# TimoLassmann/tagdust

Hardware: AMD Instinct MI355X
Metric: reads/s (150 bp, 8-barcode arch) (higher is better)
Workload: dtype f32

## Files before the change

### tagdust_amd/csrc/td_api.hip

```cpp
#include <math.h>
#include <stdarg.h>
#include <stdlib.h>
#include <string.h>
#include <time.h>
#include <unistd.h>

#include <mutex>
#include <thread>

#include "../../include/tagdust_model.h"
#include "td_ctx.h"
#include "td_rnadust.h"
#include "td_stats.h"

static float g_logsum[TD_LOGSUM_SIZE];
static bool g_logsum_ready = false;
static std::string g_create_error;

static void init_logsum_host()
{
	if (g_logsum_ready) return;
	for (int i = 0; i < TD_LOGSUM_SIZE; i++) g_logsum[i] = (float)log(1.0 + exp((double)-i / (double)1000.0f));
	g_logsum_ready = true;
}
// ... 405 lines not shown
static int slot_events(td_ctx* c, TdSlot& s)
{
	if (s.ev_k0) return TD_OK;
	HIPCHK(c, hipEventCreate(&s.ev_k0));
	HIPCHK(c, hipEventCreate(&s.ev_k1));
	HIPCHK(c, hipEventCreateWithFlags(&s.ev_up, hipEventDisableTiming));
	HIPCHK(c, hipEventCreateWithFlags(&s.ev_done, hipEventDisableTiming));
	HIPCHK(c, hipEventCreateWithFlags(&s.ev_down, hipEventDisableTiming));
	HIPCHK(c, hipEventCreateWithFlags(&s.ev_pack, hipEventDisableTiming));
	HIPCHK(c, hipEventCreateWithFlags(&s.ev_hits, hipEventDisableTiming));
	return TD_OK;
}

static void slot_release(TdSlot& s)
{
	void* dev[] = { s.d_raw, s.d_offs, s.d_read_at, s.d_keys, s.d_vals, s.d_sort_tmp, s.d_packed, s.d_lens, s.d_art_left,
	                s.d_out, s.d_res, s.d_seq, s.d_lab, s.d_keepo, s.d_rle, s.d_runs, s.d_judged };
	for (void* p : dev) if (p) (void)hipFree(p);
	void* pinned[] = { s.h_raw, s.h_offs, s.h_res, s.h_seq, s.h_lab, s.h_keepo, s.h_rle };
	for (void* p : pinned) if (p) (void)hipHostFree(p);
	hipEvent_t ev[] = { s.ev_up, s.ev_k0, s.ev_k1, s.ev_done, s.ev_down, s.ev_pack, s.ev_hits };
	for (hipEvent_t e : ev) if (e) (void)hipEventDestroy(e);
	s = TdSlot();
}

static int hbm_free(td_ctx* c, size_t& free_b)
{
	size_t total_b = 0;
	HIPCHK(c, hipMemGetInfo(&free_b, &total_b));
	return TD_OK;
}
// ... 73 lines not shown
		if (l < 0 || l > 100000) { bad = i; break; }
		if (l > lmax) lmax = (int)l;
		if (l < lmin) lmin = (int)l;
	}
	if (bad >= 0) return fail(c, "td_batch_upload: read %lld has length %lld", (long long)bad, (long long)(offs[bad + 1] - offs[bad]));
	const int64_t n_bases = n > 0 ? offs[n] - base : 0;
	const int64_t n_tiles = (n + TD_WAVE - 1) / TD_WAVE;
	const TdLengthClasses lc = plan_length_classes(offs, n, lmin, lmax, n_tiles, c->spec.ready && with_workspace && c->length_classes);
	s.n_long = lc.n_long; s.lmax_small = lc.lmax_small;
	const int nw2 = (lmax + 15) / 16, nw1 = (lmax + 31) / 32;
	const bool sorted = n > 0 && lmin != lmax;

	const size_t n_packed = (size_t)(n_tiles * (int64_t)(nw2 + nw1) * TD_WAVE), n_lanes = (size_t)(n_tiles * TD_WAVE);
	const OutLayout ol = out_layout(n_tiles, lmax, nw1);
	if (ensure(c, &s.d_raw, &s.cap_raw, (size_t)n_bases) != TD_OK || ensure(c, &s.d_offs, &s.cap_offs, (size_t)(n + 1) * 8) != TD_OK ||
	    ensure(c, &s.d_packed, &s.cap_packed, n_packed * 4) != TD_OK || ensure(c, &s.d_lens, &s.cap_lens, n_lanes * 4) != TD_OK ||
	    ensure(c, &s.d_art_left, &s.cap_art_left, n_lanes) != TD_OK || ensure(c, &s.d_out, &s.cap_out, (size_t)ol.total) != TD_OK)
		return TD_FAIL;
	size_t sort_tmp = 0;
	if (sorted) {
		sort_tmp = td_stage_sort_temp_bytes(n, lmax);
		if (ensure(c, &s.d_read_at, &s.cap_read_at, (size_t)n * 4) != TD_OK || ensure(c, &s.d_keys, &s.cap_keys, (size_t)n * 8) != TD_OK ||
		    ensure(c, &s.d_vals, &s.cap_vals, (size_t)n * 4) != TD_OK || ensure(c, &s.d_sort_tmp, &s.cap_sort_tmp, sort_tmp) != TD_OK)
			return TD_FAIL;
	}
	s.lmax = lmax; s.nw2 = nw2; s.nw1 = nw1; s.n_tiles = (int32_t)n_tiles;
	if (with_workspace && ensure_workspace(c, s) != TD_OK) { s.n_tiles = 0; return TD_FAIL; }
	s.for_spec = with_workspace && c->spec.ready;
	s.n_tiles = 0;

	const void* src = (const uint8_t*)bases + base;
	s.raw_direct = n_bases > 0 && is_pinned(src);
	if (n_bases > 0 && !s.raw_direct) {
		if (ensure_pinned(c, &s.h_raw, &s.cap_h_raw, (size_t)n_bases) != TD_OK) return TD_FAIL;
		parallel_copy(c, s.h_raw, src, (size_t)n_bases);
		src = s.h_raw;
		s.raw_host = s.h_raw;
	} else if (n_bases > 0 && c->stable_input && s.pipelined) {
		s.raw_host = (const uint8_t*)src;
	}
	HIPCHK(c, hipMemcpyAsync(s.d_offs, s.h_offs, (size_t)(n + 1) * 8, hipMemcpyHostToDevice, up));
	if (n_bases > 0) HIPCHK(c, hipMemcpyAsync(s.d_raw, src, (size_t)n_bases, hipMemcpyHostToDevice, up));
	if (up != s.aux) {
		HIPCHK(c, hipEventRecord(s.ev_up, up));
		HIPCHK(c, hipStreamWaitEvent(s.aux, s.ev_up, 0));
	}
	if (sorted)
		HIPCHK(c, td_stage_sort(s.d_offs, n, lmax, s.d_read_at, s.d_keys, s.d_keys + n, s.d_vals, s.d_sort_tmp, sort_tmp, s.aux));
	TdStageBatch& b = s.sb;
	b = TdStageBatch{};
	b.raw = s.d_raw; b.offs = s.d_offs; b.n_reads = n; b.is_ascii = is_ascii;
	b.n_tiles = (int32_t)n_tiles; b.lmax = lmax; b.nw2 = nw2; b.nw1 = nw1;
	b.read_at = sorted ? s.d_read_at : nullptr;
	b.packed = s.d_packed; b.lens = s.d_lens; b.art_left = s.d_art_left;
	b.out_soa = s.d_out; b.soa_stride = ol.soa_stride;
	b.keep = (const uint32_t*)(s.d_out + ol.keep); b.labels = (const int8_t*)(s.d_out + ol.labels);
	HIPCHK(c, td_stage_pack(b, s.aux));
	if (s.aux != s.cs) {
		HIPCHK(c, hipEventRecord(s.ev_pack, s.aux));
		HIPCHK(c, hipStreamWaitEvent(s.cs, s.ev_pack, 0));
	}

	s.n_reads = n; s.n_bases = n_bases; s.n_tiles = (int32_t)n_tiles; s.is_ascii = is_ascii; s.sorted = sorted;
	s.staged = true;
	return TD_OK;
}

static int rle_capacity(const td_ctx* c)
{
	int cap = c->dev.h.S + 2 < c->dev.h.H ? c->dev.h.S + 2 : c->dev.h.H;
	if (c->rle_cap_forced > 0) cap = c->rle_cap_forced;
	return cap;
}

static int slot_rna_dust(td_ctx* c, TdSlot& s);

static int slot_count_hits(td_ctx* c, TdSlot& s, const int32_t* out_type)
{
	HIPCHK(c, td_stage_art_hits(out_type, s.n_reads, c->art_n, c->d_art_hits, s.cs));
// ... 12 lines not shown
	HIPCHK(c, hipSetDevice(c->device));
	s.reset_decoded();
	s.mode = mode;
	if (s.n_tiles == 0) { s.ran = true; s.last_ms = 0.0f; return TD_OK; }
	if (c->spec.ready && s.for_spec && c->match_len > 0 && !c->spec.window) {
		HIPCHK(c, sync_compute(c));
		if (spec_load_window_variant(c) != TD_OK) return TD_FAIL;
		if (!c->spec.ready) {
			s.n_long = 0; s.lmax_small = s.lmax;
			if (ensure_workspace(c, s) != TD_OK) return TD_FAIL;
			s.for_spec = false;
		}
	}
	const bool use_spec = c->spec.ready && s.for_spec;
	if (s.for_spec && !c->spec.ready) return fail(c, "td_run: the resident batch was staged for a specialised kernel that is no longer loaded (upload it again)");
	const OutLayout ol = out_layout(s.n_tiles, s.lmax, s.nw1);
	TdKernelArgs ka{};
	ka.hdr = c->dev.d_hdr; ka.cols = c->dev.d_cols; ka.hinfo = c->dev.d_hinfo;
	ka.pred_off = c->dev.d_pred_off; ka.pred_idx = c->dev.d_pred_idx; ka.logsum = c->d_logsum;
	ka.packed = s.d_packed; ka.lens = s.d_lens;
	ka.n_tiles = s.n_tiles; ka.n_slots = s.n_wave_slots; ka.lmax = s.lmax; ka.nw2 = s.nw2; ka.nw1 = s.nw1;
	ka.mode = mode; ka.threshold = c->threshold; ka.minlen = c->minlen; ka.dust = c->dust; ka.want_labels = 1;
	ka.win_start = c->match_start; ka.win_len = c->match_len;
	point_outputs(ka, s.d_out, ol);
	ka.counters = c->d_counters;
	ka.ws = s.wsi ? c->d_ws2 : c->d_ws; ka.lay = s.lay;
	if (c->art_n > 0 && mode == TD_MODE_GET_LABEL) {
		s.sb.art_threads = c->art_threads;
		s.sb.art_first = c->win_first; s.sb.art_total = c->win_total;
		HIPCHK(c, td_stage_art_left(s.sb, s.cs));
		ka.art_text = c->d_art_text; ka.art_index = c->d_art_index; ka.art_left = s.d_art_left;
		ka.art_n = c->art_n; ka.art_fe = c->art_fe;
	}
	if (c->poison) HIPCHK(c, hipMemsetAsync(ka.ws, 0xFF, (size_t)s.ws_bytes, s.cs));
	if (use_spec) {
		int32_t*& tn = s.wsi ? c->d_tile_next2 : c->d_tile_next;
		if (!tn) HIPCHK(c, hipMalloc((void**)&tn, 256));
		HIPCHK(c, hipMemsetAsync(tn, 0, sizeof(int32_t), s.cs));
	}
	HIPCHK(c, hipEventRecord(s.ev_k0, s.cs));
	if (use_spec) {
		TdSpecArgs sa = spec_args_from(ka);
		sa.lay = s.slay;
		sa.lmax = s.n_big > 0 ? s.lmax_small : s.lmax;
		sa.n_big = s.n_big; sa.lmax_big = s.lmax; sa.lay_big = s.slay_big; sa.out_lmax = s.lmax;
		if (mode == TD_MODE_GET_LABEL && want_labels && c->compact_egress) {
			const int cap = rle_capacity(c);
			const size_t words = (size_t)s.n_tiles * (size_t)cap * TD_WAVE + 1;
			if (ensure(c, &s.d_runs, &s.cap_runs, words * 4) != TD_OK) return TD_FAIL;
			if (c->poison) HIPCHK(c, hipMemsetAsync(s.d_runs, 0xFF, (words - 1) * 4, s.cs));
			HIPCHK(c, hipMemsetAsync(s.d_runs + words - 1, 0, 4, s.cs));
			sa.out_runs = s.d_runs; sa.rle_overflow = (int32_t*)(s.d_runs + words - 1); sa.rle_cap = cap;
			s.runs_cap = cap;
		}
		sa.prune = c->spec.d_prune; sa.prune_stride = c->spec.prune_stride;
		sa.tile_next = s.wsi ? c->d_tile_next2 : c->d_tile_next;
		HIPCHK(c, spec_launch(c, sa, s.cs));
// ... 6 lines not shown
	if (c->census.on && mode == TD_MODE_GET_LABEL && census_count_slot(c, s, ka.out_type, ka.out_labels) != TD_OK) return TD_FAIL;
	if (c->molecules.on && mode == TD_MODE_GET_LABEL && mol_slot_decoded(c, s, ka.out_type, ka.out_barcode, ka.out_finger, ka.out_labels) != TD_OK) return TD_FAIL;
	s.ran = true;
	s.last_ms = -1.0f;
	c->last_slot = (int)(&s - c->slots);
	return TD_OK;
}

static int slot_rna_dust(td_ctx* c, TdSlot& s)
{
	if (!s.staged) return fail(c, "td_run: no batch resident (td_batch_upload failed or was not called)");
	HIPCHK(c, hipSetDevice(c->device));
	s.reset_decoded();
	s.mode = TD_MODE_RNA_DUST;
	if (s.n_tiles == 0) { s.ran = true; s.last_ms = 0.0f; return TD_OK; }
	const OutLayout ol = out_layout(s.n_tiles, s.lmax, s.nw1);
	TdRnaDustArgs ra{};
	ra.packed = s.d_packed; ra.lens = s.d_lens; ra.n_tiles = s.n_tiles; ra.nw2 = s.nw2; ra.nw1 = s.nw1;
	ra.raw = s.d_raw; ra.offs = s.d_offs; ra.read_at = s.sorted ? s.d_read_at : nullptr; ra.n_reads = s.n_reads; ra.is_ascii = s.is_ascii;
	ra.dust = c->dust;
	if (c->art_n > 0) {
		s.sb.art_threads = c->art_threads;
		s.sb.art_first = c->win_first; s.sb.art_total = c->win_total;
		HIPCHK(c, td_stage_art_left(s.sb, s.cs));
		ra.art_pk = c->d_art_pk; ra.art_seq = c->d_art_seq; ra.art_left = s.d_art_left;
		ra.art_n = c->art_n; ra.art_fe = c->art_fe;
	}
	point_outputs(ra, s.d_out, ol);
	ra.counters = c->d_counters;
	HIPCHK(c, hipEventRecord(s.ev_k0, s.cs));
// ... 452 lines not shown
```

### tagdust_amd/csrc/td_batch_plan.cpp

```cpp
#include "td_batch_plan.h"

#include <vector>

int64_t align256(int64_t v) { return (v + 255) & ~(int64_t)255; }

void make_layout(TdWsLayout& L, int S, int H, int C, int lmax, int max_ncol)
{
	int64_t o = 0;
	L.codes = o; o = align256(o + (int64_t)(lmax + 2) * TD_WAVE);
	L.sb = o;    o = align256(o + (int64_t)(S + 1) * (lmax + 2) * TD_WAVE * 4);
	L.sf = o;    o = align256(o + (int64_t)(S + 1) * (lmax + 2) * TD_WAVE * 4);
	L.bw = o;    o = align256(o + (int64_t)C * lmax * TD_WAVE * 8);
	L.fwrow = o; o = align256(o + (int64_t)max_ncol * TD_WAVE * 8);
	L.dp = o;    o = align256(o + (int64_t)lmax * H * TD_WAVE * 4);
	L.path = o;  o = align256(o + (int64_t)lmax * H * TD_WAVE);
	L.acc = o;   o = align256(o + (int64_t)H * TD_WAVE * 4);
	L.total = o; o = align256(o + (int64_t)H * TD_WAVE * 4);
	L.dust = o;  o = align256(o + (int64_t)64 * TD_WAVE);
	L.slot_bytes = o;
}

OutLayout out_layout(int64_t n_tiles, int lmax, int nw1)
{
	OutLayout o;
// ... 13 lines not shown
	for (int64_t i = 0; i < n; i++) hist[(size_t)(offs[i + 1] - offs[i])]++;
	const int64_t t99 = n_tiles - 1 - (n_tiles + 99) / 100;
	const int64_t rank = t99 * TD_WAVE + TD_WAVE - 1;
	int64_t acc = 0;
	int l99 = lmax;
	for (int l = 0; l <= lmax; l++) { acc += hist[(size_t)l]; if (acc > rank) { l99 = l; break; } }
	if (l99 < 1) l99 = 1;
	if ((int64_t)lmax * 2 >= (int64_t)l99 * 3) {
		int64_t upto = 0;
		for (int l = 0; l <= l99; l++) upto += hist[(size_t)l];
		const int64_t first_long_tile = upto / TD_WAVE;
		lc.n_long = (int32_t)(n_tiles - first_long_tile);
		lc.lmax_small = l99;
	}
	return lc;
}

TdWsPlan plan_workspace(const TdWsRequest& rq, TdFreeMemFn free_mem, void* arg)
{
	TdWsPlan p;
	p.half_slots = rq.half_slots;
	int overlap = rq.overlap, wsi = rq.wsi;
	for (;;) {
		p.n_long = rq.n_long; p.lmax_small = rq.lmax_small;
		p.one_geometry = false;
		int64_t slot_bytes = rq.small_slot_bytes;
		const int wpb = rq.wpb;
		int64_t slots = rq.want_slots;
		if (slots > rq.n_tiles) slots = rq.n_tiles;
		if (slots < 1) slots = 1;
// ... 58 lines not shown
```

### tagdust_amd/csrc/td_batch_plan.h

```cpp
#pragma once
#include <stddef.h>
#include <stdint.h>

#include "td_device.h"

#ifndef TD_HIDDEN
#define TD_HIDDEN __attribute__((visibility("hidden")))
#endif

TD_HIDDEN int64_t align256(int64_t v);
TD_HIDDEN void make_layout(TdWsLayout& L, int S, int H, int C, int lmax, int max_ncol);
struct OutLayout { int64_t soa_stride, keep, labels, total; };
TD_HIDDEN OutLayout out_layout(int64_t n_tiles, int lmax, int nw1);

struct TdLengthClasses { int32_t n_long, lmax_small; };
TD_HIDDEN TdLengthClasses plan_length_classes(const int64_t* offs, int64_t n, int lmin, int lmax, int64_t n_tiles, bool wanted);

struct TdWsRequest {
	int64_t n_tiles = 0;
	int32_t n_long = 0, lmax_small = 0, lmax = 0;
	int64_t small_slot_bytes = 0, big_slot_bytes = 0;
	int wpb = 1;
	int64_t want_slots = 0;
	bool spec_ready = false, pipelined = false;
	int overlap = 0, pipeline_depth = 1;
	bool half_slots = false;
	int wsi = 0;
	size_t cap_ws = 0, cap_ws2 = 0;
	int ws_candidates = 1;
};
struct TdWsPlan {
// ... 13 lines not shown
```

### tagdust_amd/csrc/td_ctx.h

```cpp
#pragma once
#include <hip/hip_runtime.h>
#include <stdio.h>
#include <memory>
#include <string>
#include <vector>
#include "../../include/tagdust_hip.h"
#include "td_device.h"
#include "td_batch_plan.h"
#include "td_jit.h"
#include "td_stage.h"
#include "td_host_inner.h"
#include "td_census.h"
#include "td_molecules.h"

#define TD_HIDDEN __attribute__((visibility("hidden")))
#define TD_MAX_PIPELINE 4
#define TD_COUNTER_WORDS (TD_NUM_COUNTERS + TD_NUM_DIAG_COUNTERS)

struct TdRoute {
	hipStream_t cs = nullptr;
	hipStream_t aux = nullptr;
	hipStream_t fin = nullptr;
	int wsi = 0;
	bool pipelined = false;
};
struct TdStaged : TdRoute {
	int64_t n_reads = 0, n_bases = 0;
	int32_t n_tiles = 0, lmax = 0, nw2 = 0, nw1 = 0;
	int is_ascii = 0;
	bool sorted = false;
	bool staged = false;
	bool for_spec = false;
	bool raw_direct = false;
	const uint8_t* raw_host = nullptr;
	TdStageBatch sb{};
	TdWsLayout lay{};
	TdSpecLayout slay{};
	int32_t n_wave_slots = 0;
	int64_t ws_slot_bytes = 0;
	int32_t n_long = 0, lmax_small = 0, n_big = 0;
	TdSpecLayout slay_big{};
	int64_t ws_bytes = 0;
};
struct TdDecoded {
	int mode = 0;
	bool ran = false;
	float last_ms = -1.0f;
// ... 8 lines not shown
	int32_t rle_cap = 0;
	bool finished = false;
};
struct TdSlot : TdStaged, TdDecoded, TdFetch {
	int64_t ticket = 0;
	void reset_staged(const TdRoute& r) { static_cast<TdStaged&>(*this) = TdStaged(); static_cast<TdRoute&>(*this) = r; reset_decoded(); }
	void reset_decoded() { static_cast<TdDecoded&>(*this) = TdDecoded(); reset_fetch(); }
	void reset_fetch() { static_cast<TdFetch&>(*this) = TdFetch(); }
	uint8_t* d_raw = nullptr;      size_t cap_raw = 0;
	int64_t* d_offs = nullptr;     size_t cap_offs = 0;
	int32_t* d_read_at = nullptr;  size_t cap_read_at = 0;
	uint32_t* d_keys = nullptr;    size_t cap_keys = 0;
	int32_t* d_vals = nullptr;     size_t cap_vals = 0;
	uint8_t* d_sort_tmp = nullptr; size_t cap_sort_tmp = 0;
	uint32_t* d_packed = nullptr;  size_t cap_packed = 0;
	int32_t* d_lens = nullptr;     size_t cap_lens = 0;
	uint8_t* d_art_left = nullptr; size_t cap_art_left = 0;
	uint8_t* d_out = nullptr;      size_t cap_out = 0;
	uint8_t* d_res = nullptr;      size_t cap_res = 0;
	uint8_t* d_seq = nullptr;      size_t cap_seq = 0;
	int8_t*  d_lab = nullptr;      size_t cap_lab = 0;
	uint32_t* d_keepo = nullptr;   size_t cap_keepo = 0;
	uint32_t* d_rle = nullptr;     size_t cap_rle = 0;
	uint32_t* d_runs = nullptr;    size_t cap_runs = 0;
	int32_t* d_judged = nullptr;   size_t cap_judged = 0;
	uint32_t* h_keepo = nullptr;   size_t cap_h_keepo = 0;
	uint32_t* h_rle = nullptr;     size_t cap_h_rle = 0;
	uint8_t* h_raw = nullptr;      size_t cap_h_raw = 0;
	int64_t* h_offs = nullptr;     size_t cap_h_offs = 0;
	uint8_t* h_res = nullptr;      size_t cap_h_res = 0;
// ... 163 lines not shown
template <typename Args> static void point_labels(Args&, int8_t*, long) {}
template <typename Args>
static void point_outputs(Args& a, uint8_t* out, const OutLayout& ol)
{
	float* soa = (float*)out;
	const int64_t st = ol.soa_stride / 4;
	a.out_f = soa; a.out_b = soa + st; a.out_r = soa + 2 * st; a.out_bar = soa + 3 * st; a.out_q = soa + 4 * st;
	a.out_type = (int32_t*)(soa + 5 * st); a.out_barcode = (int32_t*)(soa + 6 * st); a.out_finger = (int32_t*)(soa + 7 * st);
	a.out_keep = (uint32_t*)(out + ol.keep);
	point_labels(a, (int8_t*)(out + ol.labels), 0);
}

static TdSpecArgs spec_args_from(const TdKernelArgs& ka)
{
	TdSpecArgs sa{};
	sa.logsum = ka.logsum; sa.packed = ka.packed; sa.lens = ka.lens;
	sa.n_tiles = ka.n_tiles; sa.n_slots = ka.n_slots; sa.lmax = ka.lmax; sa.nw2 = ka.nw2; sa.nw1 = ka.nw1;
	sa.mode = ka.mode; sa.threshold = ka.threshold; sa.minlen = ka.minlen; sa.dust = ka.dust;
	sa.win_start = ka.win_start; sa.win_len = ka.win_len;
	sa.out_f = ka.out_f; sa.out_b = ka.out_b; sa.out_r = ka.out_r; sa.out_bar = ka.out_bar; sa.out_q = ka.out_q;
	sa.out_type = ka.out_type; sa.out_barcode = ka.out_barcode; sa.out_finger = ka.out_finger;
	sa.out_keep = ka.out_keep; sa.out_labels = ka.out_labels; sa.counters = ka.counters;
	sa.art_text = ka.art_text; sa.art_index = ka.art_index; sa.art_left = ka.art_left; sa.art_n = ka.art_n; sa.art_fe = ka.art_fe;
	sa.ws = ka.ws;
	return sa;
}

TD_HIDDEN int spec_model_uploaded(td_ctx* c);
TD_HIDDEN int spec_handover(td_ctx* c, bool block);
TD_HIDDEN int spec_before_batch(td_ctx* c, int lmax);
TD_HIDDEN int spec_load_window_variant(td_ctx* c);
// ... 5 lines not shown
```

### tagdust_amd/csrc/td_device.h

```cpp
#pragma once
#include <stdint.h>

#define TD_WAVE 64
#define TD_LOGSUM_LIVE 15700

enum : uint32_t {
	TDF_MM = 1u << 0, TDF_MI = 1u << 1, TDF_MD = 1u << 2, TDF_II = 1u << 3, TDF_IM = 1u << 4,
	TDF_DD = 1u << 5, TDF_DM = 1u << 6, TDF_MSKIP = 1u << 7, TDF_ISKIP = 1u << 8,
	TDF_SM = 1u << 9, TDF_SI = 1u << 10,
};

struct TdCol {
	float    t[9];
	float    sM, sI;
	float    eM[5];
	float    eI[5];
	uint32_t flags;
	uint32_t pad[2];
};
static_assert(sizeof(TdCol) == 96, "TdCol layout");

struct TdSeg {
	int32_t n_hmm, n_col, col_off, hmm_off;
	float   skip;
// ... 49 lines not shown
	float*   __restrict__ out_q;
	int32_t* __restrict__ out_type;
	int32_t* __restrict__ out_barcode;
	int32_t* __restrict__ out_finger;
	uint32_t* __restrict__ out_keep;
	int8_t*  __restrict__ out_labels;
	unsigned long long* __restrict__ counters;
	const uint8_t*  __restrict__ art_text;
	const int32_t*  __restrict__ art_index;
	const uint8_t*  __restrict__ art_left;
	int32_t art_n, art_fe;
	uint8_t* __restrict__ ws;
	TdWsLayout lay;
};

struct TdSpecLayout {
	int64_t slot_bytes;
	int64_t codes;
	int64_t sb;
	int64_t sf;
	int64_t bw;
	int64_t dp;
	int64_t path;
	int64_t total;
	int64_t rs;
	int64_t bm;
	int64_t ba;
	int64_t acc;
	int64_t pmask;
};

struct TdSpecArgs {
	const float*  __restrict__ logsum;
	const uint32_t* __restrict__ packed;
	const int32_t*  __restrict__ lens;
	int32_t n_tiles, n_slots, lmax, nw2, nw1;
	int32_t mode;
	float   threshold;
	int32_t minlen, dust;
	int32_t win_start, win_len;
	int32_t prune_stride;
	float*   __restrict__ out_f;
	float*   __restrict__ out_b;
	float*   __restrict__ out_r;
	float*   __restrict__ out_bar;
	float*   __restrict__ out_q;
	int32_t* __restrict__ out_type;
	int32_t* __restrict__ out_barcode;
	int32_t* __restrict__ out_finger;
	uint32_t* __restrict__ out_keep;
// ... 18 lines not shown
```

### tagdust_amd/csrc/td_jit.hip

```cpp
#include <hip/hip_runtime.h>
#include <hip/hiprtc.h>
#include <math.h>
#include <stdio.h>
#include <string.h>
#include <stdlib.h>

#include <atomic>
#include <map>
#include <mutex>
#include <string>
#include <vector>

#include "../../include/tagdust_hip.h"
#include "td_device.h"
#include <unistd.h>
#include <sys/stat.h>
#include <sys/types.h>
#include "td_embedded_src.h"
#include "td_jit.h"

static std::string flit(float v)
{
	if (isinf(v)) return v < 0 ? "(-__builtin_inff())" : "__builtin_inff()";
	if (v != v) return "__builtin_nanf(\"\")";
// ... 285 lines not shown
{
	std::string src = "#ifndef __HIPCC_RTC__\n#include <hip/hip_runtime.h>\n#endif\n#include <stdint.h>\n";
	src += kSrcDeviceH;
	src += "\n";
	src += kSrcArtifact;
	src += "\n";
	src += td_spec_model_section(m, p, lsum_oob, window);
	src += kSrcSpecKernel;
	return src;
}

void td_spec_layout(TdSpecLayout& L, const TdSpecPlan& p, int lmax)
{
	auto al = [](int64_t v) { return (v + 255) & ~(int64_t)255; };
	int64_t o = 0;
	L.codes = o; o = al(o + (int64_t)(lmax + 2) * TD_WAVE);
	L.sb = o;    o = al(o + (int64_t)(p.S + 1) * (lmax + 2) * TD_WAVE * 4);
	L.sf = o;    o = al(o + (int64_t)(p.S + 1) * (lmax + 2) * TD_WAVE * 4);
	L.bw = o;    o = al(o + p.halves * lmax * TD_WAVE * 4 + 1024);
	L.dp = o;    o = al(o + (int64_t)lmax * p.H * TD_WAVE * 4);
	L.path = o;  o = al(o + (int64_t)lmax * ((p.H + 3) / 4) * TD_WAVE * 4);
	L.total = o; o = al(o + (int64_t)p.H * TD_WAVE * 4);
	L.rs = o;    o = al(o + (int64_t)2 * p.C * TD_WAVE * 4);
	L.bm = o;    o = al(o + (int64_t)(lmax + 2) * TD_WAVE * 4);
	L.ba = o;    o = al(o + (int64_t)(lmax + 2) * TD_WAVE);
	L.acc = o;   o = al(o + (int64_t)2 * p.H * TD_WAVE * 4);
	L.pmask = o; o = al(o + (int64_t)p.H * ((lmax + 31) / 32) * 4);
	L.slot_bytes = o;
}

static uint64_t fnv1a(const std::string& t)
// ... 171 lines not shown
```

### tagdust_amd/csrc/td_spec_host.hip

```cpp
#include <stdlib.h>
#include <algorithm>
#include <cmath>
#include <condition_variable>
#include <map>
#include <mutex>
#include <thread>

#include "td_ctx.h"

struct SpecJob {
	uint64_t key = 0;
	ModelCopy model;
	TdSpecPlan plan;
	int lsum_oob = 0, window = 0;
	std::mutex mu;
	std::condition_variable cv;
	bool done = false;
	int rc = TD_FAIL;
	std::vector<char> code;
	std::string log;
	std::thread th;
	void run()
	{
		std::vector<char> out;
// ... 70 lines not shown
	std::vector<uint8_t> codes((size_t)n_bases);
	(void)td_spec_probe(&c->model.d, codes.data(), n_bases, nullptr);
	const int n = TD_PROBE_READS, n_tiles = TD_PROBE_READS / TD_WAVE;
	int lmax = 1;
	for (int i = 0; i < n; i++) if (offs[(size_t)i + 1] - offs[(size_t)i] > lmax) lmax = (int)(offs[(size_t)i + 1] - offs[(size_t)i]);
	const int nw2 = (lmax + 15) / 16, nw1 = (lmax + 31) / 32;
	if (ensure_prune_tables(c, lmax) != TD_OK) return TD_FAIL;
	const TdModelHeader& h = c->dev.h;
	TdWsLayout glay{};
	make_layout(glay, h.S, h.H, h.C, lmax, h.max_ncol);
	TdSpecLayout slay{};
	td_spec_layout(slay, c->spec.plan, lmax);
	const int gwpb = td_kernel_block_threads() / TD_WAVE, swpb = c->spec.block / TD_WAVE;
	const int gslots = (n_tiles + gwpb - 1) / gwpb * gwpb, sslots = (n_tiles + swpb - 1) / swpb * swpb;
	const OutLayout ol = out_layout(n_tiles, lmax, nw1);
	int64_t o = 0;
	auto carve = [&](int64_t bytes) { const int64_t at = o; o = align256(o + bytes); return at; };
	const int64_t o_raw = carve(n_bases), o_offs = carve((int64_t)(n + 1) * 8), o_packed = carve((int64_t)n_tiles * (nw2 + nw1) * TD_WAVE * 4),
	              o_lens = carve((int64_t)n * 4), o_outa = carve(ol.total), o_outb = carve(ol.total),
	              o_cnt = carve((int64_t)2 * TD_COUNTER_WORDS * 8), o_cmp = carve(256), o_tile = carve(256);
	const int64_t small_bytes = o;
	const int64_t o_wsa = carve((int64_t)gslots * glay.slot_bytes), o_wsb = carve((int64_t)sslots * slay.slot_bytes);
	uint8_t* d = nullptr;
	HIPCHK(c, hipMalloc((void**)&d, (size_t)o));
	struct Free { uint8_t* p; ~Free() { (void)hipFree(p); } } free_{ d };
	hipStream_t st = c->stream;
	HIPCHK(c, hipMemsetAsync(d, 0, (size_t)small_bytes, st));
	HIPCHK(c, hipMemsetAsync(d + o_cmp, 0xFF, 256, st));
	HIPCHK(c, hipMemsetAsync(d + o_cmp, 0, 4, st));
	HIPCHK(c, hipMemsetAsync(d + o_wsa, 0xFF, (size_t)(o - o_wsa), st));
	HIPCHK(c, hipMemcpyAsync(d + o_raw, codes.data(), (size_t)n_bases, hipMemcpyHostToDevice, st));
	HIPCHK(c, hipMemcpyAsync(d + o_offs, offs.data(), (size_t)(n + 1) * 8, hipMemcpyHostToDevice, st));
	TdStageBatch sb{};
	sb.raw = d + o_raw; sb.offs = (const int64_t*)(d + o_offs); sb.n_reads = n; sb.is_ascii = 0;
	sb.n_tiles = n_tiles; sb.lmax = lmax; sb.nw2 = nw2; sb.nw1 = nw1;
	sb.read_at = nullptr;
	sb.packed = (uint32_t*)(d + o_packed); sb.lens = (int32_t*)(d + o_lens);
	HIPCHK(c, td_stage_pack(sb, st));
	unsigned long long* cnt_a = (unsigned long long*)(d + o_cnt);
	unsigned long long* cnt_b = cnt_a + TD_COUNTER_WORDS;
	TdKernelArgs ka{};
	ka.hdr = c->dev.d_hdr; ka.cols = c->dev.d_cols; ka.hinfo = c->dev.d_hinfo; ka.pred_off = c->dev.d_pred_off; ka.pred_idx = c->dev.d_pred_idx; ka.logsum = c->d_logsum;
	ka.packed = sb.packed; ka.lens = sb.lens;
	ka.n_tiles = n_tiles; ka.n_slots = gslots; ka.lmax = lmax; ka.nw2 = nw2; ka.nw1 = nw1;
	ka.mode = TD_MODE_GET_LABEL; ka.threshold = TD_PROBE_THRESHOLD; ka.minlen = TD_PROBE_MINLEN; ka.dust = TD_PROBE_DUST; ka.want_labels = 1;
	if (window) { ka.win_start = TD_PROBE_WIN_START; ka.win_len = TD_PROBE_WIN_END - TD_PROBE_WIN_START; }
	point_outputs(ka, d + o_outa, ol);
	ka.counters = cnt_a;
	ka.ws = d + o_wsa; ka.lay = glay;
	HIPCHK(c, td_launch_decode(&ka, st));
	TdSpecArgs sa = spec_args_from(ka);
	sa.n_slots = sslots;
	point_outputs(sa, d + o_outb, ol);
	sa.counters = cnt_b;
	sa.ws = d + o_wsb; sa.lay = slay; sa.lay_big = slay;
	sa.n_big = 0; sa.lmax_big = lmax; sa.out_lmax = lmax;
	sa.prune = c->spec.d_prune; sa.prune_stride = c->spec.prune_stride;
	sa.tile_next = (int32_t*)(d + o_tile);
	HIPCHK(c, spec_launch(c, sa, st));
	TdProbeCmp pc{};
	pc.lens = sb.lens; pc.n_tiles = n_tiles; pc.lmax = lmax; pc.nw1 = nw1; pc.n_counters = TD_NUM_COUNTERS;
	pc.soa_a = d + o_outa; pc.soa_b = d + o_outb; pc.soa_stride = ol.soa_stride;
	pc.keep_a = ka.out_keep; pc.keep_b = sa.out_keep; pc.labels_a = ka.out_labels; pc.labels_b = sa.out_labels;
	pc.counters_a = cnt_a; pc.counters_b = cnt_b;
	pc.out = (int32_t*)(d + o_cmp);
	HIPCHK(c, td_probe_compare(pc, st));
	int32_t out[1 + 2 * (TD_PROBE_READS / TD_WAVE + 1)];
// ... 198 lines not shown
```

### tagdust_amd/csrc/td_spec_kernel.inc

```

#ifndef TDS_BLOCK
#define TDS_BLOCK 512
#endif
#ifndef TDS_MIN_WAVES
#define TDS_MIN_WAVES 4
#endif
#define TDS_REG_H 32
#define TDS_WPB (TDS_BLOCK / TD_WAVE)
#define NEG_INF (-__builtin_inff())
#define DEV __device__ __forceinline__

#define MODE_GET_LABEL 1
#define MODE_ARCH_COMP 5
#define OUT_SUCCESS 0
#define OUT_ARCH_MISMATCH 1
#define OUT_TOO_SHORT 2
#define OUT_BAR_FINGER_NOT_FOUND 3
#define OUT_MATCHES_ARTIFACTS 5
#define OUT_LOW_COMPLEXITY 6
#define N_OUTCOME_SLOTS 8
#define TDS_DIAG(k) (N_OUTCOME_SLOTS + 256 + ((k) - 192))

#ifndef TDS_LSUM_OOB
#define TDS_LSUM_OOB 1
// ... 1334 lines not shown
	const bool big = slot < ka.n_big;
	const TdSpecLayout& lay = big ? ka.lay_big : ka.lay;
	const int lmax = big ? ka.lmax_big : ka.lmax;
	const int rowlen = (lmax + 2) * TD_WAVE;
	constexpr int PW = (TD_H + 3) / 4;

	Wv w;
	w.slot = big ? ka.ws + (int64_t)slot * ka.lay_big.slot_bytes
	             : ka.ws + (int64_t)ka.n_big * ka.lay_big.slot_bytes + (int64_t)(slot - ka.n_big) * ka.lay.slot_bytes;
	w.lane = lane;
	w.lmax = lmax;
	w.pmask = (uint32_t*)(w.slot + lay.pmask);
	w.nwm = (lmax + 31) >> 5;
	w.bm = (float*)(w.slot + lay.bm);
	w.ba = w.slot + lay.ba;
	uint8_t* const codesF = w.slot + lay.codes;
	float* SB = (float*)(w.slot + lay.sb);
	float* SF = (float*)(w.slot + lay.sf);
	uint8_t* BW = w.slot + lay.bw;
	float* DP = (float*)(w.slot + lay.dp);
	uint32_t* PATH = (uint32_t*)(w.slot + lay.path);
	float* TOTAL = (float*)(w.slot + lay.total);

#ifdef TDS_ENDSTATS
	const unsigned long long t_start = wall_clock64();
#endif
	long long tprof = TDS_PROFILE ? (long long)__builtin_readcyclecounter() : 0;
	(void)tprof;
	int n_fallback = 0, n_tiles_done = 0;
	bool prune_on = true;
	bool restart_on = true;
// ... 45 lines not shown
		for (int o = 32; o >= 1; o >>= 1) tmax = max(tmax, __shfl_xor(tmax, o));
		tmax = __builtin_amdgcn_readfirstlane(tmax);
		w.tmax = tmax;
		int tmin = len;
#pragma unroll
		for (int o = 32; o >= 1; o >>= 1) tmin = min(tmin, __shfl_xor(tmin, o));
		w.tmin = __builtin_amdgcn_readfirstlane(tmin);
#if TDS_WINDOW
		int tmaxF = lenF;
#pragma unroll
		for (int o = 32; o >= 1; o >>= 1) tmaxF = max(tmaxF, __shfl_xor(tmaxF, o));
		tmaxF = __builtin_amdgcn_readfirstlane(tmaxF);
#else
		const int tmaxF = tmax;
#endif
		uint8_t* const codes = codesF + woff * TD_WAVE;

		TDS_PHASE(11);
		float r_score = 0.0f;
		{
			const uint32_t* pk = ka.packed + (int64_t)tile * (ka.nw2 + ka.nw1) * TD_WAVE;
			codesF[lane] = 0;
			uint32_t w2 = 0, w1 = 0;
			uint32_t w2n = (ka.nw2 > 0) ? pk[lane] : 0u, w1n = (ka.nw1 > 0) ? pk[ka.nw2 * TD_WAVE + lane] : 0u;
			for (int i = 1; i <= tmaxF + 1; i++) {
				const int k = i - 1;
				if ((k & 15) == 0) { w2 = w2n; w2n = ((k >> 4) + 1) < ka.nw2 ? pk[((k >> 4) + 1) * TD_WAVE + lane] : 0u; }
				if ((k & 31) == 0) { w1 = w1n; w1n = ((k >> 5) + 1) < ka.nw1 ? pk[(ka.nw2 + (k >> 5) + 1) * TD_WAVE + lane] : 0u; }
				uint32_t code = (w2 >> (2 * (k & 15))) & 3u;
				if ((w1 >> (k & 31)) & 1u) code = 4u;
				if (i > lenF) code = 0u;
				codesF[i * TD_WAVE + lane] = (uint8_t)code;
				const int iw = i - woff;
				if (iw >= 1 && iw <= len) r_score = (r_score + emit(kBg[0], kBg[1], kBg[2], kBg[3], kBg[4], mk_mask((int)code))) + kRStay;
			}
		}

		TDS_PHASE(0);
		r_score += kRExit;

		float b_score = NEG_INF, f_score = NEG_INF, b_use = 0.0f;
		bool dead = false, arch_done = false;
		bool dense = !((kPruneSegs > 0 || kSfxFirst < TD_S) && prune_on);
		int cut_guess = tmax;
		if (kPruneSegs > 0 && !dense)
			cut_guess = prune_scan((len >= 1 ? r_score : 0.0f) - bgap - kPruneZ, len, tmax, ka.prune, ka.prune + ka.prune_stride) + 1 + TDS_PRUNE_MARGIN;
		int sfx_guess = 1;
		if (kSfxFirst < TD_S && !dense) {
			sfx_guess = prune_scan_sfx((len >= 1 ? r_score : 0.0f) - bgap - kPruneZ, len, tmax, ka.prune + 4 * (int64_t)ka.prune_stride,
			                           ka.prune + 5 * (int64_t)ka.prune_stride) - TDS_PRUNE_MARGIN;
			if (sfx_guess < 1) sfx_guess = 1;
// ... 713 lines not shown
```

### tagdust_amd/csrc/td_stage.h

```cpp
#pragma once
#include <hip/hip_runtime.h>
#include <stdint.h>

struct TdStageBatch {
	const uint8_t* raw;
	const int64_t* offs;
	int64_t n_reads;
	int32_t is_ascii;
	int32_t n_tiles, lmax, nw2, nw1;
	const int32_t* read_at;
	int32_t art_threads;
	int64_t art_first, art_total;
	uint32_t* packed;
	int32_t*  lens;
	uint8_t*  art_left;
	const uint8_t* out_soa;
	int64_t   soa_stride;
	const uint32_t* keep;
	const int8_t*  labels;
	const uint32_t* runs;
	uint8_t* res;
	uint8_t* seq_out;
	int8_t*  labels_out;
	uint32_t* keep_out;
	uint32_t* rle_out;
	int32_t   rle_cap;
	int32_t*  rle_overflow;
	const int32_t* runs_overflow;
// ... 23 lines not shown
```

### tagdust_amd/csrc/td_stage.hip

```cpp
#include <hip/hip_runtime.h>
#include <string.h>
#include <rocprim/device/device_radix_sort.hpp>

#include "td_device.h"
#include "td_stage.h"

#define STAGE_BLOCK 256

__global__ __launch_bounds__(STAGE_BLOCK) void td_len_iota_kernel(const int64_t* __restrict__ offs, int64_t n,
                                                                    uint32_t* __restrict__ keys, int32_t* __restrict__ vals)
{
	const int64_t i = (int64_t)blockIdx.x * STAGE_BLOCK + threadIdx.x;
	if (i >= n) return;
	keys[i] = (uint32_t)(offs[i + 1] - offs[i]);
	vals[i] = (int32_t)i;
}

static int key_bits(int lmax)
{
	int b = 1;
	while (b < 32 && ((int64_t)1 << b) <= (int64_t)lmax) b++;
	return b;
}

// ... 50 lines not shown
		const int p0 = c * 32;
		const int e = len - p0 < 32 ? len - p0 : 32;
		for (int q = 0; q < e; q++) {
			const uint32_t cd = base_code(src[p0 + q], b.is_ascii);
			if (cd == 4u) w1 |= 1u << q;
			else if (q < 16) w2a |= cd << (2 * q);
			else w2b |= cd << (2 * (q - 16));
		}
		pk[(2 * c) * TD_WAVE + lane] = w2a;
		if (2 * c + 1 < b.nw2) pk[(2 * c + 1) * TD_WAVE + lane] = w2b;
		pk[(b.nw2 + c) * TD_WAVE + lane] = w1;
	}
	if (wv == 0) b.lens[k] = len;
}

__global__ __launch_bounds__(STAGE_BLOCK) void td_art_left_kernel(const TdStageBatch b)
{
	const int64_t k = (int64_t)blockIdx.x * STAGE_BLOCK + threadIdx.x;
	if (k >= (int64_t)b.n_tiles * TD_WAVE) return;
	uint8_t left = 0;
	if (k < b.n_reads && b.art_threads > 0) {
		const int64_t i = b.art_first + (b.read_at ? (int64_t)b.read_at[k] : k);
		const int64_t n = b.art_total > 0 ? b.art_total : b.n_reads, T = b.art_threads, interval = n / T;
		int64_t t = interval > 0 ? i / interval : T - 1;
		if (t > T - 1) t = T - 1;
		const int64_t start = t * interval, end = (t == T - 1) ? n : (t + 1) * interval;
		left = i >= start + (end - start) / 4 * 4;
	}
	b.art_left[k] = left;
}
// ... 27 lines not shown
		if (bin[i]) atomicAdd(hits + i, (unsigned long long)bin[i]);
}

hipError_t td_stage_art_hits(const int32_t* out_type, int64_t n_reads, int32_t art_n, unsigned long long* hits, hipStream_t stream)
{
	if (n_reads <= 0 || art_n <= 0) return hipSuccess;
	int64_t blocks = (n_reads + STAGE_BLOCK * 8 - 1) / (STAGE_BLOCK * 8);
	if (blocks > 1024) blocks = 1024;
	hipLaunchKernelGGL(td_art_hits_kernel, dim3((unsigned)blocks), dim3(STAGE_BLOCK), 0, stream, out_type, n_reads, art_n, hits);
	return hipGetLastError();
}

hipError_t td_stage_pack(const TdStageBatch& b, hipStream_t stream)
{
	if (b.n_tiles <= 0) return hipSuccess;
	hipLaunchKernelGGL(td_pack_kernel, dim3((unsigned)b.n_tiles), dim3(STAGE_BLOCK), 0, stream, b);
	return hipGetLastError();
}

__global__ __launch_bounds__(STAGE_BLOCK) void td_finish_kernel(const TdStageBatch b)
{
	const int tile = blockIdx.x;
	__shared__ int64_t s_off[TD_WAVE];
	__shared__ int64_t s_idx[TD_WAVE];
	__shared__ int32_t s_len[TD_WAVE];
	if (threadIdx.x < TD_WAVE) {
		const int lane = threadIdx.x;
		const int64_t k = (int64_t)tile * TD_WAVE + lane;
		int64_t i = -1, o = 0;
		int len = -1;
		if (k < b.n_reads) {
// ... 170 lines not shown
```

Measured before the change: 83.68 million.

## Precompute byte codes and random-model score in staging kernel for specialised decode

Adds a staging kernel that expands reads into a per-tile byte-code array in global memory and precomputes the random-model score per read. The specialised decode kernel then reads these codes directly, instead of unpacking 2-bit words into its per-slot workspace and accumulating the score itself. The 2-bit packing is skipped unless census, molecule or rna-dust paths need it, and is built lazily when they do. This trades more staging work and global memory (one byte per base) for less per-tile work inside the decode kernel.

```diff
diff --git a/tagdust_amd/csrc/td_api.hip b/tagdust_amd/csrc/td_api.hip
--- a/tagdust_amd/csrc/td_api.hip
+++ b/tagdust_amd/csrc/td_api.hip
@@ -443,7 +443,7 @@
 
 static void slot_release(TdSlot& s)
 {
-	void* dev[] = { s.d_raw, s.d_offs, s.d_read_at, s.d_keys, s.d_vals, s.d_sort_tmp, s.d_packed, s.d_lens, s.d_art_left,
+	void* dev[] = { s.d_raw, s.d_offs, s.d_read_at, s.d_keys, s.d_vals, s.d_sort_tmp, s.d_packed, s.d_codes8, s.d_rsum, s.d_lens, s.d_art_left,
 	                s.d_out, s.d_res, s.d_seq, s.d_lab, s.d_keepo, s.d_rle, s.d_runs, s.d_judged };
 	for (void* p : dev) if (p) (void)hipFree(p);
 	void* pinned[] = { s.h_raw, s.h_offs, s.h_res, s.h_seq, s.h_lab, s.h_keepo, s.h_rle };
@@ -547,7 +547,7 @@
 	const size_t n_packed = (size_t)(n_tiles * (int64_t)(nw2 + nw1) * TD_WAVE), n_lanes = (size_t)(n_tiles * TD_WAVE);
 	const OutLayout ol = out_layout(n_tiles, lmax, nw1);
 	if (ensure(c, &s.d_raw, &s.cap_raw, (size_t)n_bases) != TD_OK || ensure(c, &s.d_offs, &s.cap_offs, (size_t)(n + 1) * 8) != TD_OK ||
-	    ensure(c, &s.d_packed, &s.cap_packed, n_packed * 4) != TD_OK || ensure(c, &s.d_lens, &s.cap_lens, n_lanes * 4) != TD_OK ||
+	    ensure(c, &s.d_lens, &s.cap_lens, n_lanes * 4) != TD_OK ||
 	    ensure(c, &s.d_art_left, &s.cap_art_left, n_lanes) != TD_OK || ensure(c, &s.d_out, &s.cap_out, (size_t)ol.total) != TD_OK)
 		return TD_FAIL;
 	size_t sort_tmp = 0;
@@ -561,6 +561,11 @@
 	if (with_workspace && ensure_workspace(c, s) != TD_OK) { s.n_tiles = 0; return TD_FAIL; }
 	s.for_spec = with_workspace && c->spec.ready;
 	s.n_tiles = 0;
+	const bool want_packed = !s.for_spec || c->census.on || c->molecules.on;
+	const TdCodesGeo geo = plan_codes8(n_tiles, s.n_long, s.lmax_small, lmax);
+	if (want_packed && ensure(c, &s.d_packed, &s.cap_packed, n_packed * 4) != TD_OK) return TD_FAIL;
+	if (s.for_spec && (ensure(c, &s.d_codes8, &s.cap_codes8, (size_t)geo.total) != TD_OK || ensure(c, &s.d_rsum, &s.cap_rsum, n_lanes * 4) != TD_OK))
+		return TD_FAIL;
 
 	const void* src = (const uint8_t*)bases + base;
 	s.raw_direct = n_bases > 0 && is_pinned(src);
@@ -585,7 +590,12 @@
 	b.raw = s.d_raw; b.offs = s.d_offs; b.n_reads = n; b.is_ascii = is_ascii;
 	b.n_tiles = (int32_t)n_tiles; b.lmax = lmax; b.nw2 = nw2; b.nw1 = nw1;
 	b.read_at = sorted ? s.d_read_at : nullptr;
-	b.packed = s.d_packed; b.lens = s.d_lens; b.art_left = s.d_art_left;
+	b.packed = want_packed ? s.d_packed : nullptr; b.lens = s.d_lens; b.art_left = s.d_art_left;
+	if (s.for_spec) {
+		b.codes8 = s.d_codes8; b.r_sum = s.d_rsum; b.codes_geo = geo;
+		for (int i = 0; i < 5; i++) b.bg[i] = c->dev.h.bg[i];
+		b.r_stay = c->dev.h.r_stay;
+	}
 	b.out_soa = s.d_out; b.soa_stride = ol.soa_stride;
 	b.keep = (const uint32_t*)(s.d_out + ol.keep); b.labels = (const int8_t*)(s.d_out + ol.labels);
 	HIPCHK(c, td_stage_pack(b, s.aux));
@@ -595,7 +605,20 @@
 	}
 
 	s.n_reads = n; s.n_bases = n_bases; s.n_tiles = (int32_t)n_tiles; s.is_ascii = is_ascii; s.sorted = sorted;
+	s.packed_ready = want_packed;
 	s.staged = true;
+	return TD_OK;
+}
+
+static int slot_need_packed(td_ctx* c, TdSlot& s)
+{
+	if (s.packed_ready || s.n_tiles == 0) return TD_OK;
+	if (ensure(c, &s.d_packed, &s.cap_packed, (size_t)s.n_tiles * (size_t)(s.nw2 + s.nw1) * TD_WAVE * 4) != TD_OK) return TD_FAIL;
+	TdStageBatch b = s.sb;
+	b.packed = s.d_packed; b.codes8 = nullptr; b.r_sum = nullptr;
+	HIPCHK(c, td_stage_pack(b, s.cs));
+	s.sb.packed = s.d_packed;
+	s.packed_ready = true;
 	return TD_OK;
 }
 
@@ -638,6 +661,7 @@
 	}
 	const bool use_spec = c->spec.ready && s.for_spec;
 	if (s.for_spec && !c->spec.ready) return fail(c, "td_run: the resident batch was staged for a specialised kernel that is no longer loaded (upload it again)");
+	if ((!use_spec || ((c->census.on || c->molecules.on) && mode == TD_MODE_GET_LABEL)) && slot_need_packed(c, s) != TD_OK) return TD_FAIL;
 	const OutLayout ol = out_layout(s.n_tiles, s.lmax, s.nw1);
 	TdKernelArgs ka{};
 	ka.hdr = c->dev.d_hdr; ka.cols = c->dev.d_cols; ka.hinfo = c->dev.d_hinfo;
@@ -665,6 +689,7 @@
 	HIPCHK(c, hipEventRecord(s.ev_k0, s.cs));
 	if (use_spec) {
 		TdSpecArgs sa = spec_args_from(ka);
+		sa.codes8 = s.sb.codes8; sa.r_sum = s.sb.r_sum; sa.codes_geo = s.sb.codes_geo;
 		sa.lay = s.slay;
 		sa.lmax = s.n_big > 0 ? s.lmax_small : s.lmax;
 		sa.n_big = s.n_big; sa.lmax_big = s.lmax; sa.lay_big = s.slay_big; sa.out_lmax = s.lmax;
@@ -701,6 +726,7 @@
 	s.reset_decoded();
 	s.mode = TD_MODE_RNA_DUST;
 	if (s.n_tiles == 0) { s.ran = true; s.last_ms = 0.0f; return TD_OK; }
+	if (slot_need_packed(c, s) != TD_OK) return TD_FAIL;
 	const OutLayout ol = out_layout(s.n_tiles, s.lmax, s.nw1);
 	TdRnaDustArgs ra{};
 	ra.packed = s.d_packed; ra.lens = s.d_lens; ra.n_tiles = s.n_tiles; ra.nw2 = s.nw2; ra.nw1 = s.nw1;
diff --git a/tagdust_amd/csrc/td_batch_plan.cpp b/tagdust_amd/csrc/td_batch_plan.cpp
--- a/tagdust_amd/csrc/td_batch_plan.cpp
+++ b/tagdust_amd/csrc/td_batch_plan.cpp
@@ -51,6 +51,21 @@
 		lc.lmax_small = l99;
 	}
 	return lc;
+}
+
+TdCodesGeo plan_codes8(int64_t n_tiles, int32_t n_long, int32_t lmax_small, int32_t lmax)
+{
+	TdCodesGeo g{};
+	if (n_long < 0) n_long = 0;
+	if (n_long > n_tiles) n_long = (int32_t)n_tiles;
+	if (n_long == 0) lmax_small = lmax;
+	if (n_long == n_tiles && n_tiles > 0) lmax_small = lmax;
+	g.first_long = (int32_t)(n_tiles - n_long);
+	g.lmax = lmax_small; g.lmax_big = lmax;
+	g.stride = (int64_t)(lmax_small + 2) * TD_WAVE;
+	g.stride_big = (int64_t)(lmax + 2) * TD_WAVE;
+	g.total = (int64_t)g.first_long * g.stride + (int64_t)n_long * g.stride_big;
+	return g;
 }
 
 TdWsPlan plan_workspace(const TdWsRequest& rq, TdFreeMemFn free_mem, void* arg)
diff --git a/tagdust_amd/csrc/td_batch_plan.h b/tagdust_amd/csrc/td_batch_plan.h
--- a/tagdust_amd/csrc/td_batch_plan.h
+++ b/tagdust_amd/csrc/td_batch_plan.h
@@ -15,6 +15,8 @@
 
 struct TdLengthClasses { int32_t n_long, lmax_small; };
 TD_HIDDEN TdLengthClasses plan_length_classes(const int64_t* offs, int64_t n, int lmin, int lmax, int64_t n_tiles, bool wanted);
+
+TD_HIDDEN TdCodesGeo plan_codes8(int64_t n_tiles, int32_t n_long, int32_t lmax_small, int32_t lmax);
 
 struct TdWsRequest {
 	int64_t n_tiles = 0;
diff --git a/tagdust_amd/csrc/td_ctx.h b/tagdust_amd/csrc/td_ctx.h
--- a/tagdust_amd/csrc/td_ctx.h
+++ b/tagdust_amd/csrc/td_ctx.h
@@ -31,6 +31,7 @@
 	bool sorted = false;
 	bool staged = false;
 	bool for_spec = false;
+	bool packed_ready = false;
 	bool raw_direct = false;
 	const uint8_t* raw_host = nullptr;
 	TdStageBatch sb{};
@@ -69,6 +70,8 @@
 	int32_t* d_vals = nullptr;     size_t cap_vals = 0;
 	uint8_t* d_sort_tmp = nullptr; size_t cap_sort_tmp = 0;
 	uint32_t* d_packed = nullptr;  size_t cap_packed = 0;
+	uint8_t* d_codes8 = nullptr;   size_t cap_codes8 = 0;
+	float* d_rsum = nullptr;       size_t cap_rsum = 0;
 	int32_t* d_lens = nullptr;     size_t cap_lens = 0;
 	uint8_t* d_art_left = nullptr; size_t cap_art_left = 0;
 	uint8_t* d_out = nullptr;      size_t cap_out = 0;
@@ -262,7 +265,7 @@
 static TdSpecArgs spec_args_from(const TdKernelArgs& ka)
 {
 	TdSpecArgs sa{};
-	sa.logsum = ka.logsum; sa.packed = ka.packed; sa.lens = ka.lens;
+	sa.logsum = ka.logsum; sa.lens = ka.lens;
 	sa.n_tiles = ka.n_tiles; sa.n_slots = ka.n_slots; sa.lmax = ka.lmax; sa.nw2 = ka.nw2; sa.nw1 = ka.nw1;
 	sa.mode = ka.mode; sa.threshold = ka.threshold; sa.minlen = ka.minlen; sa.dust = ka.dust;
 	sa.win_start = ka.win_start; sa.win_len = ka.win_len;
diff --git a/tagdust_amd/csrc/td_device.h b/tagdust_amd/csrc/td_device.h
--- a/tagdust_amd/csrc/td_device.h
+++ b/tagdust_amd/csrc/td_device.h
@@ -87,9 +87,32 @@
 	TdWsLayout lay;
 };
 
+struct TdCodesGeo {
+	int32_t first_long;
+	int32_t lmax, lmax_big;
+	int32_t pad;
+	int64_t stride, stride_big, total;
+};
+#if defined(__HIP__) || defined(__HIPCC__) || defined(__HIPCC_RTC__)
+#define TD_HOST_DEVICE __host__ __device__
+#else
+#define TD_HOST_DEVICE
+#endif
+TD_HOST_DEVICE static inline int64_t td_codes8_offset(const TdCodesGeo& g, int tile)
+{
+	return tile < g.first_long ? (int64_t)tile * g.stride : (int64_t)g.first_long * g.stride + (int64_t)(tile - g.first_long) * g.stride_big;
+}
+TD_HOST_DEVICE static inline float td_r_sum_step(float r, uint32_t code, float bg0, float bg1, float bg2, float bg3, float bg4, float stay)
+{
+#if defined(__clang__)
+#pragma clang fp contract(off) reassociate(off)
+#endif
+	const float e = code == 0u ? bg0 : code == 1u ? bg1 : code == 2u ? bg2 : code == 3u ? bg3 : bg4;
+	return (r + e) + stay;
+}
+
 struct TdSpecLayout {
 	int64_t slot_bytes;
-	int64_t codes;
 	int64_t sb;
 	int64_t sf;
 	int64_t bw;
@@ -105,8 +128,10 @@
 
 struct TdSpecArgs {
 	const float*  __restrict__ logsum;
-	const uint32_t* __restrict__ packed;
+	const uint8_t* __restrict__ codes8;
+	const float*  __restrict__ r_sum;
 	const int32_t*  __restrict__ lens;
+	TdCodesGeo codes_geo;
 	int32_t n_tiles, n_slots, lmax, nw2, nw1;
 	int32_t mode;
 	float   threshold;
diff --git a/tagdust_amd/csrc/td_jit.hip b/tagdust_amd/csrc/td_jit.hip
--- a/tagdust_amd/csrc/td_jit.hip
+++ b/tagdust_amd/csrc/td_jit.hip
@@ -323,7 +323,6 @@
 {
 	auto al = [](int64_t v) { return (v + 255) & ~(int64_t)255; };
 	int64_t o = 0;
-	L.codes = o; o = al(o + (int64_t)(lmax + 2) * TD_WAVE);
 	L.sb = o;    o = al(o + (int64_t)(p.S + 1) * (lmax + 2) * TD_WAVE * 4);
 	L.sf = o;    o = al(o + (int64_t)(p.S + 1) * (lmax + 2) * TD_WAVE * 4);
 	L.bw = o;    o = al(o + p.halves * lmax * TD_WAVE * 4 + 1024);
diff --git a/tagdust_amd/csrc/td_spec_host.hip b/tagdust_amd/csrc/td_spec_host.hip
--- a/tagdust_amd/csrc/td_spec_host.hip
+++ b/tagdust_amd/csrc/td_spec_host.hip
@@ -108,10 +108,11 @@
 	const int gwpb = td_kernel_block_threads() / TD_WAVE, swpb = c->spec.block / TD_WAVE;
 	const int gslots = (n_tiles + gwpb - 1) / gwpb * gwpb, sslots = (n_tiles + swpb - 1) / swpb * swpb;
 	const OutLayout ol = out_layout(n_tiles, lmax, nw1);
+	const TdCodesGeo geo = plan_codes8(n_tiles, 0, lmax, lmax);
 	int64_t o = 0;
 	auto carve = [&](int64_t bytes) { const int64_t at = o; o = align256(o + bytes); return at; };
 	const int64_t o_raw = carve(n_bases), o_offs = carve((int64_t)(n + 1) * 8), o_packed = carve((int64_t)n_tiles * (nw2 + nw1) * TD_WAVE * 4),
-	              o_lens = carve((int64_t)n * 4), o_outa = carve(ol.total), o_outb = carve(ol.total),
+	              o_lens = carve((int64_t)n * 4), o_codes8 = carve(geo.total), o_rsum = carve((int64_t)n * 4), o_outa = carve(ol.total), o_outb = carve(ol.total),
 	              o_cnt = carve((int64_t)2 * TD_COUNTER_WORDS * 8), o_cmp = carve(256), o_tile = carve(256);
 	const int64_t small_bytes = o;
 	const int64_t o_wsa = carve((int64_t)gslots * glay.slot_bytes), o_wsb = carve((int64_t)sslots * slay.slot_bytes);
@@ -130,6 +131,9 @@
 	sb.n_tiles = n_tiles; sb.lmax = lmax; sb.nw2 = nw2; sb.nw1 = nw1;
 	sb.read_at = nullptr;
 	sb.packed = (uint32_t*)(d + o_packed); sb.lens = (int32_t*)(d + o_lens);
+	sb.codes8 = d + o_codes8; sb.r_sum = (float*)(d + o_rsum); sb.codes_geo = geo;
+	for (int i = 0; i < 5; i++) sb.bg[i] = h.bg[i];
+	sb.r_stay = h.r_stay;
 	HIPCHK(c, td_stage_pack(sb, st));
 	unsigned long long* cnt_a = (unsigned long long*)(d + o_cnt);
 	unsigned long long* cnt_b = cnt_a + TD_COUNTER_WORDS;
@@ -145,6 +149,7 @@
 	HIPCHK(c, td_launch_decode(&ka, st));
 	TdSpecArgs sa = spec_args_from(ka);
 	sa.n_slots = sslots;
+	sa.codes8 = sb.codes8; sa.r_sum = sb.r_sum; sa.codes_geo = geo;
 	point_outputs(sa, d + o_outb, ol);
 	sa.counters = cnt_b;
 	sa.ws = d + o_wsb; sa.lay = slay; sa.lay_big = slay;
diff --git a/tagdust_amd/csrc/td_spec_kernel.inc b/tagdust_amd/csrc/td_spec_kernel.inc
--- a/tagdust_amd/csrc/td_spec_kernel.inc
+++ b/tagdust_amd/csrc/td_spec_kernel.inc
@@ -1372,7 +1372,6 @@
 	w.nwm = (lmax + 31) >> 5;
 	w.bm = (float*)(w.slot + lay.bm);
 	w.ba = w.slot + lay.ba;
-	uint8_t* const codesF = w.slot + lay.codes;
 	float* SB = (float*)(w.slot + lay.sb);
 	float* SF = (float*)(w.slot + lay.sf);
 	uint8_t* BW = w.slot + lay.bw;
@@ -1448,27 +1447,17 @@
 #else
 		const int tmaxF = tmax;
 #endif
-		uint8_t* const codes = codesF + woff * TD_WAVE;
+		const uint8_t* const codesF = ka.codes8 + td_codes8_offset(ka.codes_geo, tile);
+		const uint8_t* const codes = codesF + (woff <= tmaxF ? woff : tmaxF) * TD_WAVE;
 
 		TDS_PHASE(11);
+#if TDS_WINDOW
 		float r_score = 0.0f;
-		{
-			const uint32_t* pk = ka.packed + (int64_t)tile * (ka.nw2 + ka.nw1) * TD_WAVE;
-			codesF[lane] = 0;
-			uint32_t w2 = 0, w1 = 0;
-			uint32_t w2n = (ka.nw2 > 0) ? pk[lane] : 0u, w1n = (ka.nw1 > 0) ? pk[ka.nw2 * TD_WAVE + lane] : 0u;
-			for (int i = 1; i <= tmaxF + 1; i++) {
-				const int k = i - 1;
-				if ((k & 15) == 0) { w2 = w2n; w2n = ((k >> 4) + 1) < ka.nw2 ? pk[((k >> 4) + 1) * TD_WAVE + lane] : 0u; }
-				if ((k & 31) == 0) { w1 = w1n; w1n = ((k >> 5) + 1) < ka.nw1 ? pk[(ka.nw2 + (k >> 5) + 1) * TD_WAVE + lane] : 0u; }
-				uint32_t code = (w2 >> (2 * (k & 15))) & 3u;
-				if ((w1 >> (k & 31)) & 1u) code = 4u;
-				if (i > lenF) code = 0u;
-				codesF[i * TD_WAVE + lane] = (uint8_t)code;
-				const int iw = i - woff;
-				if (iw >= 1 && iw <= len) r_score = (r_score + emit(kBg[0], kBg[1], kBg[2], kBg[3], kBg[4], mk_mask((int)code))) + kRStay;
-			}
-		}
+		for (int i = 1; i <= tmax; i++)
+			if (i <= len) r_score = (r_score + emit(kBg[0], kBg[1], kBg[2], kBg[3], kBg[4], mk_mask((int)codes[i * TD_WAVE + lane]))) + kRStay;
+#else
+		float r_score = ka.r_sum[rid];
+#endif
 
 		TDS_PHASE(0);
 		r_score += kRExit;
diff --git a/tagdust_amd/csrc/td_stage.h b/tagdust_amd/csrc/td_stage.h
--- a/tagdust_amd/csrc/td_stage.h
+++ b/tagdust_amd/csrc/td_stage.h
@@ -1,6 +1,8 @@
 #pragma once
 #include <hip/hip_runtime.h>
 #include <stdint.h>
+
+#include "td_device.h"
 
 struct TdStageBatch {
 	const uint8_t* raw;
@@ -12,6 +14,10 @@
 	int32_t art_threads;
 	int64_t art_first, art_total;
 	uint32_t* packed;
+	uint8_t*  codes8;
+	float*    r_sum;
+	TdCodesGeo codes_geo;
+	float     bg[5], r_stay;
 	int32_t*  lens;
 	uint8_t*  art_left;
 	const uint8_t* out_soa;
diff --git a/tagdust_amd/csrc/td_stage.hip b/tagdust_amd/csrc/td_stage.hip
--- a/tagdust_amd/csrc/td_stage.hip
+++ b/tagdust_amd/csrc/td_stage.hip
@@ -88,6 +88,72 @@
 	if (wv == 0) b.lens[k] = len;
 }
 
+#define CODES_CHUNK 128
+__device__ __forceinline__ uint32_t read_bases4(const uint8_t* src, int at, int len)
+{
+	if (at >= len) return 0u;
+	const uintptr_t a = (uintptr_t)(src + at);
+	const uint32_t* al = (const uint32_t*)(a & ~(uintptr_t)3);
+	const int sh = (int)(a & 3);
+	uint32_t v = al[0] >> (8 * sh);
+	if (sh && at + (4 - sh) < len) v |= al[1] << (32 - 8 * sh);
+	const int have = len - at;
+	return have >= 4 ? v : v & ((1u << (8 * have)) - 1u);
+}
+
+__global__ __launch_bounds__(STAGE_BLOCK) void td_codes_kernel(const TdStageBatch b)
+{
+	__shared__ __attribute__((aligned(16))) uint8_t s_codes[CODES_CHUNK * TD_WAVE];
+	const int tile = blockIdx.x;
+	const int lane = threadIdx.x & (TD_WAVE - 1);
+	const int wv = threadIdx.x >> 6;
+	const int64_t k = (int64_t)tile * TD_WAVE + lane;
+	int len = 0;
+	const uint8_t* src = nullptr;
+	if (k < b.n_reads) {
+		const int64_t i = b.read_at ? (int64_t)b.read_at[k] : k;
+		const int64_t o = b.offs[i];
+		len = (int)(b.offs[i + 1] - o);
+		src = b.raw + o;
+	}
+	const int n_after = (tile < b.codes_geo.first_long ? b.codes_geo.lmax : b.codes_geo.lmax_big) + 1;
+	uint8_t* dst = b.codes8 + td_codes8_offset(b.codes_geo, tile);
+	if (threadIdx.x < TD_WAVE / 16) ((uint4*)dst)[threadIdx.x] = make_uint4(0u, 0u, 0u, 0u);
+	const float bg0 = b.bg[0], bg1 = b.bg[1], bg2 = b.bg[2], bg3 = b.bg[3], bg4 = b.bg[4], stay = b.r_stay;
+	float r = 0.0f;
+	constexpr int PER_WAVE = CODES_CHUNK / (STAGE_BLOCK / TD_WAVE);
+	for (int b0 = 0; b0 < n_after; b0 += CODES_CHUNK) {
+		const int n = n_after - b0 < CODES_CHUNK ? n_after - b0 : CODES_CHUNK;
+		uint32_t w4[PER_WAVE / 4];
+#pragma unroll
+		for (int g = 0; g < PER_WAVE / 4; g++) w4[g] = read_bases4(src, b0 + wv * PER_WAVE + 4 * g, len);
+#pragma unroll
+		for (int g = 0; g < PER_WAVE / 4; g++) {
+#pragma unroll
+			for (int j = 0; j < 4; j++) {
+				const int q = wv * PER_WAVE + 4 * g + j;
+				if (q < n) s_codes[q * TD_WAVE + lane] = b0 + q < len ? (uint8_t)base_code((w4[g] >> (8 * j)) & 0xFFu, b.is_ascii) : (uint8_t)0;
+			}
+		}
+		__syncthreads();
+		const uint4* s4 = (const uint4*)s_codes;
+		uint4* d4 = (uint4*)(dst + (int64_t)(b0 + 1) * TD_WAVE);
+		for (int t = threadIdx.x; t < n * (TD_WAVE / 16); t += STAGE_BLOCK) d4[t] = s4[t];
+		if (wv == 0) {
+#pragma unroll 8
+			for (int q = 0; q < n; q++) {
+				const float r1 = td_r_sum_step(r, s_codes[q * TD_WAVE + lane], bg0, bg1, bg2, bg3, bg4, stay);
+				r = b0 + q < len ? r1 : r;
+			}
+		}
+		__syncthreads();
+	}
+	if (wv == 0) {
+		b.r_sum[k] = r;
+		if (!b.packed) b.lens[k] = len;
+	}
+}
+
 __global__ __launch_bounds__(STAGE_BLOCK) void td_art_left_kernel(const TdStageBatch b)
 {
 	const int64_t k = (int64_t)blockIdx.x * STAGE_BLOCK + threadIdx.x;
@@ -145,7 +211,9 @@
 hipError_t td_stage_pack(const TdStageBatch& b, hipStream_t stream)
 {
 	if (b.n_tiles <= 0) return hipSuccess;
-	hipLaunchKernelGGL(td_pack_kernel, dim3((unsigned)b.n_tiles), dim3(STAGE_BLOCK), 0, stream, b);
+	if (!b.packed && !(b.codes8 && b.r_sum)) return hipErrorInvalidValue;
+	if (b.packed) hipLaunchKernelGGL(td_pack_kernel, dim3((unsigned)b.n_tiles), dim3(STAGE_BLOCK), 0, stream, b);
+	if (b.codes8 && b.r_sum) hipLaunchKernelGGL(td_codes_kernel, dim3((unsigned)b.n_tiles), dim3(STAGE_BLOCK), 0, stream, b);
 	return hipGetLastError();
 }
 
```

After: 81.67 million. -2.4%, worse.
